# OATML-Markslab/ProteinGym

Hardware: AMD Instinct MI355X
Metric: mutants scored/sec (ESM-1v 650M masked-marginal) (higher is better)
Workload: dtype f16x3 (fp32 operands split into 2 fp16 planes, 3 fp16 MFMAs per product, fp32 accumulate)

## Files before the change

proteingym_amd/csrc/gemm16x_kernel.h:

```cpp
#pragma once
#include <type_traits>

#include "common.h"

namespace pgmi {

typedef _Float16 h8 __attribute__((ext_vector_type(8)));
typedef _Float16 h4 __attribute__((ext_vector_type(4)));
typedef __bf16 b8 __attribute__((ext_vector_type(8)));
typedef unsigned int u32x4 __attribute__((ext_vector_type(4)));
typedef unsigned int u32x2 __attribute__((ext_vector_type(2)));

__device__ __forceinline__ f32x4 gelu_erf16(f32x4 x) {
    auto all = [](float v) { return f32x4{v, v, v, v}; };
    const f32x4 b = __builtin_elementwise_max(-__builtin_elementwise_abs(x), all(-6.0f));
    f32x4 q = __builtin_elementwise_fma(x, all(0.0f), all(3.309269596e-05f));
    q = __builtin_elementwise_fma(q, b, all(7.692188374e-04f));
    q = __builtin_elementwise_fma(q, b, all(8.080714382e-03f));
    q = __builtin_elementwise_fma(q, b, all(5.341210216e-02f));
    q = __builtin_elementwise_fma(q, b, all(-4.587709904e-01f));
    q = __builtin_elementwise_fma(q, b, all(1.151201725e+00f));
    q = __builtin_elementwise_fma(q, b, all(-9.999930859e-01f));
    const f32x4 e = {__builtin_amdgcn_exp2f(q[0]), __builtin_amdgcn_exp2f(q[1]), __builtin_amdgcn_exp2f(q[2]), __builtin_amdgcn_exp2f(q[3])};
    return __builtin_elementwise_fma(b, e, __builtin_elementwise_max(x, all(0.0f)));
}

__device__ __forceinline__ f32x4 gelu_tanh16(f32x4 x) {
    constexpr float c = -2.0f * 0.7978845608028654f * 1.4426950408889634f;
    f32x4 r;
#pragma unroll
    for (int e = 0; e < 4; ++e) {
        const float u = fmaf(0.044715f * x[e], x[e] * x[e], x[e]);
        r[e] = x[e] / (1.0f + __builtin_amdgcn_exp2f(c * u));
    }
    return r;
}

struct QkvOut {
    unsigned short* vt16;
    size_t vt_plane;
    const float* cos_t;
    const float* sin_t;
    int T, H, Tp, rotary;
    int rot_halves;
};

template <bool BF>
__device__ __forceinline__ f32x16 mfma16(u32x4 a, u32x4 b, f32x16 c) {
    if constexpr (BF) {
        return __builtin_amdgcn_mfma_f32_32x32x16_bf16(__builtin_bit_cast(b8, a), __builtin_bit_cast(b8, b), c, 0, 0, 0);
    } else {
        return __builtin_amdgcn_mfma_f32_32x32x16_f16(__builtin_bit_cast(h8, a), __builtin_bit_cast(h8, b), c, 0, 0, 0);
    }
}

__device__ __forceinline__ unsigned short f32_to_bf16_rne(float f) {
    unsigned int u = __builtin_bit_cast(unsigned int, f);
    u += 0x7fffu + ((u >> 16) & 1u);
    return (unsigned short)(u >> 16);
}

struct TilePlan {
    int tiles_m, tiles_n;
    int n_main;
    int n_tail;
    int half;
    int group_m;
};

struct XMap {
    unsigned int a_row_bytes, w_row_bytes;
    unsigned int a_bytes, w_bytes;
    int k_run_log2;
    unsigned int a_run_bytes, w_run_bytes;
    int tiles_per_batch, batch_inner;
    unsigned int a_b0, a_b1, w_b0, w_b1;
    long long c_b0, c_b1;
    int ldc;
    int o_ld;
    int o_rows_per_n64;
    int o_col_per_batch;
};

constexpr int XBM = 256, XBN = 256, XNT = 512, XCPR = 8;
constexpr int X_OP_CH = XBM * XCPR;
constexpr int X_STAGE = 2 * X_OP_CH;
constexpr int X_PATCH_BYTES = 72 * 1024;
constexpr size_t X_LDS_BYTES = (size_t)(X_STAGE * 16 + X_PATCH_BYTES);

__device__ __forceinline__ void x_tile_coords(int wgid, int tiles_m, int tiles_n, int& tm, int& tn, int GROUP_M) {
    const int width = GROUP_M * tiles_n;
    const int group = wgid / width, first_m = group * GROUP_M;
    const int gsz = min(tiles_m - first_m, GROUP_M);
    tm = first_m + (wgid % width) % gsz;
    tn = (wgid % width) / gsz;
}

template <int EPI, int OUT, bool XM = false, bool BF = false>
__global__ __launch_bounds__(XNT, 2) void gemm16x_kernel(
    const unsigned short* __restrict__ A, const unsigned short* __restrict__ W, const float* __restrict__ bias,
    const float* residual, float* Cf, unsigned short* Ch, size_t c_plane, int M, int N, int K, float out_scale,
    TilePlan tp, QkvOut qo, XMap xm_arg) {
    static_assert(!(XM && BF), "the batched / strided form is f16x3 only");
    constexpr unsigned int EB = BF ? 2u : 4u;
    const XMap xm = XM ? xm_arg : XMap{};
    constexpr int WN = 4, TMX = 4, TN = 2, LD = 4;
    extern __shared__ __attribute__((aligned(16))) u32x4 lds[];
    const int tid = threadIdx.x, lane = tid & 63;
    const int wave = __builtin_amdgcn_readfirstlane(tid >> 6);
    const int wm = wave / WN, wn = wave % WN;
    const int r = lane & 31, kh = lane >> 5;
    const bool late = wave >= 4;
    unsigned char* const patches = reinterpret_cast<unsigned char*>(lds + X_STAGE);

    const int row_lo = tid >> 3, c8 = tid & 7, sw8 = (row_lo >> 1) & 7;
    const int csrc = c8 ^ sw8;
    const unsigned int a_row_bytes = xm.a_row_bytes ? xm.a_row_bytes : (unsigned int)K * EB;
    const unsigned int w_row_bytes = xm.w_row_bytes ? xm.w_row_bytes : (unsigned int)K * EB;
    const __amdgpu_buffer_rsrc_t rsA = __builtin_amdgcn_make_buffer_rsrc(const_cast<unsigned short*>(A), 0, (int)(xm.a_bytes ? xm.a_bytes : (unsigned int)M * (unsigned int)K * EB), 0x00020000);
    const __amdgpu_buffer_rsrc_t rsW = __builtin_amdgcn_make_buffer_rsrc(const_cast<unsigned short*>(W), 0, (int)(xm.w_bytes ? xm.w_bytes : (unsigned int)N * (unsigned int)K * EB), 0x00020000);
    unsigned int a_off[LD], w_off[LD];
    int m0 = 0, n0 = 0, a_ld = LD, batch = 0;
    unsigned int a_base = 0, w_base = 0;
    bool half_item = false;
    const int nk = BF ? K / 64 : K / 32;
    const int n_items = tp.n_main + tp.n_tail;
    auto decode = [&](int item) {
        const bool all_half = tp.half == 2;
        int wgid;
        if (item < tp.n_main || all_half) {
            const int nwg = all_half ? n_items : tp.n_main, xcd = item & 7, q = nwg >> 3, r8 = nwg & 7;
            wgid = (xcd < r8 ? xcd * (q + 1) : r8 * (q + 1) + (xcd - r8) * q) + (item >> 3);
        } else {
            wgid = tp.n_main + ((item - tp.n_main) >> 1);
        }
        batch = 0;
        if (xm.tiles_per_batch) {
            batch = wgid / xm.tiles_per_batch;
            wgid -= batch * xm.tiles_per_batch;
            const int bi = batch % xm.batch_inner, bo = batch / xm.batch_inner;
            a_base = __builtin_amdgcn_readfirstlane((unsigned int)bi * xm.a_b0 + (unsigned int)bo * xm.a_b1);
            w_base = __builtin_amdgcn_readfirstlane((unsigned int)bi * xm.w_b0 + (unsigned int)bo * xm.w_b1);
            batch = __builtin_amdgcn_readfirstlane(batch);
        }
        int tm, tn;
        x_tile_coords(wgid, tp.tiles_m, tp.tiles_n, tm, tn, tp.group_m);
        half_item = all_half || (tp.half && item >= tp.n_main);
        a_ld = half_item ? LD / 2 : LD;
        m0 = __builtin_amdgcn_readfirstlane(all_half ? tm * (XBM / 2) : tm * XBM + (half_item ? ((item - tp.n_main) & 1) * (XBM / 2) : 0));
        n0 = __builtin_amdgcn_readfirstlane(tn * XBN);
#pragma unroll
        for (int i = 0; i < LD; ++i) {
            a_off[i] = (unsigned int)min(m0 + row_lo + 64 * i, M - 1) * a_row_bytes + (unsigned int)csrc * 16u;
            w_off[i] = (unsigned int)min(n0 + row_lo + 64 * i, N - 1) * w_row_bytes + (unsigned int)csrc * 16u;
        }
    };
    auto issue_tile = [&](int kt, int buf) {
        u32x4* base = lds + buf * X_STAGE + wave * 64;
        const int run = kt >> xm.k_run_log2, in_run = kt - (run << xm.k_run_log2);
        const int ka = (int)(a_base + (xm.a_run_bytes ? (unsigned int)run * xm.a_run_bytes + (unsigned int)in_run * 128u : (unsigned int)kt * 128u));
        const int kw = (int)(w_base + (xm.w_run_bytes ? (unsigned int)run * xm.w_run_bytes + (unsigned int)in_run * 128u : (unsigned int)kt * 128u));
#pragma unroll
        for (int i = 0; i < LD; ++i)
            if (i < a_ld)
                __builtin_amdgcn_raw_ptr_buffer_load_lds(rsA, (__attribute__((address_space(3))) void*)(base + XNT * i), 16, (int)a_off[i], ka, 0, 0);
#pragma unroll
        for (int i = 0; i < LD; ++i)
            __builtin_amdgcn_raw_ptr_buffer_load_lds(rsW, (__attribute__((address_space(3))) void*)(base + X_OP_CH + XNT * i), 16, (int)w_off[i], kw, 0, 0);
    };
    auto phase = [&]() {
        __builtin_amdgcn_sched_barrier(0);
        __builtin_amdgcn_s_waitcnt(0xC07F);
        __builtin_amdgcn_s_barrier();
        __builtin_amdgcn_sched_barrier(0);
    };
    auto phase_vm = [&]() {
        __builtin_amdgcn_sched_barrier(0);
        __builtin_amdgcn_s_waitcnt(0x0070);
        __builtin_amdgcn_s_barrier();
        __builtin_amdgcn_sched_barrier(0);
    };

    f32x16 acc[TN][TMX];
    u32x4 af[2][TMX], wf[2][TN], whs[TN];
    const int fsw = (r >> 1) & 7;
    auto read_frags = [&](auto tmc, const u32x4* Ab, const u32x4* Wb, int ks) {
        constexpr int TM = decltype(tmc)::value;
#pragma unroll
        for (int p = 0; p < 2; ++p) {
            const int c = (p * 4 + ks * 2 + kh) ^ fsw;
#pragma unroll
            for (int i = 0; i < TM; ++i) af[p][i] = Ab[((wm * TM + i) * 32 + r) * XCPR + c];
#pragma unroll
            for (int j = 0; j < TN; ++j) wf[p][j] = Wb[((wn * TN + j) * 32 + r) * XCPR + c];
        }
    };
    auto scale_whi = [&]() {
        typedef _Float16 h2 __attribute__((ext_vector_type(2)));
        const h2 sc = {(_Float16)(1.0f / kLoScale), (_Float16)(1.0f / kLoScale)};
#pragma unroll
        for (int j = 0; j < TN; ++j)
#pragma unroll
            for (int e = 0; e < 4; ++e) {
                const unsigned int u = wf[0][j][e];
                const h2 t = __builtin_bit_cast(h2, u) * sc;
                whs[j][e] = __builtin_bit_cast(unsigned int, t);
            }
    };
    auto mfmas = [&](auto tmc) {
        constexpr int TM = decltype(tmc)::value;
        if constexpr (BF) {
#pragma unroll
            for (int p = 0; p < 2; ++p)
#pragma unroll
                for (int j = 0; j < TN; ++j)
#pragma unroll
                    for (int i = 0; i < TM; ++i) acc[j][i] = mfma16<true>(wf[p][j], af[p][i], acc[j][i]);
            return;
        }
        scale_whi();
#pragma unroll
        for (int j = 0; j < TN; ++j)
#pragma unroll
            for (int i = 0; i < TM; ++i) acc[j][i] = mfma16<false>(wf[1][j], af[0][i], acc[j][i]);
#pragma unroll
        for (int j = 0; j < TN; ++j)
#pragma unroll
            for (int i = 0; i < TM; ++i) acc[j][i] = mfma16<false>(whs[j], af[1][i], acc[j][i]);
#pragma unroll
        for (int j = 0; j < TN; ++j)
#pragma unroll
            for (int i = 0; i < TM; ++i) acc[j][i] = mfma16<false>(wf[0][j], af[0][i], acc[j][i]);
#pragma unroll
        for (int k = 0; k < 8; ++k) {
            __builtin_amdgcn_sched_group_barrier(0x008, 1, 0);
            __builtin_amdgcn_sched_group_barrier(0x002, 1, 0);
        }
        __builtin_amdgcn_sched_group_barrier(0x008, 3 * TN * TM - 8, 0);
    };

    int item = blockIdx.x;
    if (item >= n_items) return;
    decode(item);
    issue_tile(0, 0);
    auto run_item = [&](auto tmc) -> bool {
        constexpr int TM = decltype(tmc)::value;
        phase_vm();
#pragma unroll
        for (int j = 0; j < TN; ++j)
#pragma unroll
            for (int i = 0; i < TM; ++i)
#pragma unroll
                for (int v = 0; v < 16; ++v) acc[j][i][v] = 0.0f;
        int cur = 0;
        if (late) phase();
        for (int kt = 0; kt < nk; ++kt) {
            const u32x4* Ab = lds + cur * X_STAGE;
            const u32x4* Wb = Ab + X_OP_CH;
            __builtin_amdgcn_s_setprio(0);
            if (kt + 1 < nk) issue_tile(kt + 1, cur ^ 1);
            read_frags(tmc, Ab, Wb, 0);
            phase();
            __builtin_amdgcn_s_setprio(1);
            mfmas(tmc);
            phase();
            __builtin_amdgcn_s_setprio(0);
            read_frags(tmc, Ab, Wb, 1);
            if (late) phase_vm(); else phase();
            __builtin_amdgcn_s_setprio(1);
            mfmas(tmc);
            if (!late) phase_vm(); else phase();
            cur ^= 1;
        }
        __builtin_amdgcn_s_setprio(0);
        if (!late) phase();

        const int em0 = m0, en0 = n0, eb = batch;
        item += gridDim.x;
        const bool more = item < n_items;
        if (more) {
            decode(item);
            issue_tile(0, 0);
        }

        if constexpr (OUT == 2) {
            const int Dm = N / 3;
            const int nb = en0 + wn * 64;
            if (nb < N) {
            const int which = nb / Dm, hcol = nb - which * Dm, hh = hcol >> 6;
            constexpr int SPQ = 144;
            unsigned char* patch_q = patches + wave * (2 * 32 * SPQ);
            const bool staged_q = which < 2;
            f32x4 bq0[4], bq1[4];
#pragma unroll
            for (int g = 0; g < 4; ++g) {
                bq0[g] = *reinterpret_cast<const f32x4*>(bias + nb + 8 * g + 4 * kh);
                bq1[g] = *reinterpret_cast<const f32x4*>(bias + nb + 32 + 8 * g + 4 * kh);
            }
#pragma unroll
            for (int g = 0; g < 4; ++g) asm volatile("" :: "v"(bq0[g]), "v"(bq1[g]));
#pragma unroll
            for (int i = 0; i < TM; ++i) {
                const int m = em0 + (wm * TM + i) * 32 + r;
                const bool row_ok = m < M;
                if (!staged_q && !row_ok) continue;
                const int bb = m / qo.T, t = m - bb * qo.T;
                f32x4 rc[4], rs[4];
                if (which < 2 && qo.rotary) {
                    const int tr = (min(t, qo.T - 1) * qo.rot_halves + (hh % qo.rot_halves)) * 64;
#pragma unroll
                    for (int g = 0; g < 4; ++g) {
                        rc[g] = *reinterpret_cast<const f32x4*>(qo.cos_t + tr + 8 * g + 4 * kh);
                        rs[g] = *reinterpret_cast<const f32x4*>(qo.sin_t + tr + 8 * g + 4 * kh);
                    }
                }
                if (row_ok)
#pragma unroll
                for (int g = 0; g < 4; ++g) {
                    const int d0 = 8 * g + 4 * kh;
                    const f32x4 b0 = bq0[g], b1 = bq1[g];
                    float x0[4], x1[4];
#pragma unroll
                    for (int e = 0; e < 4; ++e) {
                        x0[e] = fmaf(acc[0][i][4 * g + e], out_scale, b0[e]);
                        x1[e] = fmaf(acc[1][i][4 * g + e], out_scale, b1[e]);
                    }
                    if (which == 0) {
#pragma unroll
                        for (int e = 0; e < 4; ++e) { x0[e] *= kQLog2e; x1[e] *= kQLog2e; }
                    }
                    if (which < 2) {
                        if (qo.rotary) {
                            const f32x4 c1 = rc[g], s1 = rs[g], c2 = rc[g], s2 = rs[g];
#pragma unroll
                            for (int e = 0; e < 4; ++e) {
                                const float y0 = fmaf(x0[e], c1[e], (-x1[e]) * s1[e]);
                                const float y1 = fmaf(x1[e], c2[e], x0[e] * s2[e]);
                                x0[e] = y0;
                                x1[e] = y1;
                            }
                        }
                        h4 hi0, lo0, hi1, lo1;
#pragma unroll
                        for (int e = 0; e < 4; ++e) {
                            _Float16 a, b2;
                            split_act(x0[e], a, b2); hi0[e] = a; lo0[e] = b2;
                            split_act(x1[e], a, b2); hi1[e] = a; lo1[e] = b2;
                        }
                        unsigned char* cell = patch_q + r * SPQ + d0 * 2;
                        *reinterpret_cast<h4*>(cell) = hi0;
                        *reinterpret_cast<h4*>(cell + 32 * SPQ) = lo0;
                        *reinterpret_cast<h4*>(cell + 64) = hi1;
                        *reinterpret_cast<h4*>(cell + 32 * SPQ + 64) = lo1;
                    } else {
                        const int tk = t & 31;
                        const int pos = (t & ~31) + ((tk & 0x13) | ((tk & 4) << 1) | ((tk & 8) >> 1));
                        unsigned short* col = qo.vt16 + (((size_t)bb * qo.H + hh) * kHeadDim + d0) * qo.Tp + pos;
#pragma unroll
                        for (int e = 0; e < 4; ++e) {
                            _Float16 a0, l0, a1, l1;
                            split_act(x0[e], a0, l0);
                            split_act(x1[e], a1, l1);
                            unsigned short* c0 = col + (size_t)e * qo.Tp;
                            unsigned short* c1p = c0 + (size_t)32 * qo.Tp;
                            c0[0] = __builtin_bit_cast(unsigned short, a0);
                            c0[qo.vt_plane] = __builtin_bit_cast(unsigned short, l0);
                            c1p[0] = __builtin_bit_cast(unsigned short, a1);
                            c1p[qo.vt_plane] = __builtin_bit_cast(unsigned short, l1);
                        }
                    }
                }
                if (staged_q) {
                    __builtin_amdgcn_wave_barrier();
                    const int m_base = em0 + (wm * TM + i) * 32;
#pragma unroll
                    for (int k = 0; k < 4; ++k) {
                        const int q = lane + 64 * k, row = q >> 3, cc = q & 7;
                        const u32x4 vh = *reinterpret_cast<const u32x4*>(patch_q + row * SPQ + cc * 16);
                        const u32x4 vl = *reinterpret_cast<const u32x4*>(patch_q + (32 + row) * SPQ + cc * 16);
                        if (m_base + row < M) {
                            unsigned short* dst = Ch + (size_t)(m_base + row) * (2 * Dm) + (size_t)which * Dm + hcol + cc * 8;
                            *reinterpret_cast<u32x4*>(dst) = vh;
                            *reinterpret_cast<u32x4*>(dst + c_plane) = vl;
                        }
                    }
                    __builtin_amdgcn_wave_barrier();
                }
            }
            }
        } else if constexpr (OUT == 0) {
            unsigned char* patch = patches + wave * (32 * 128);
            const int cc = lane & 7, rq = lane >> 3;
            const unsigned int kOob = 0x80000000u;
            const unsigned int ldc = xm.ldc ? (unsigned int)xm.ldc : (unsigned int)N;
            const long long cb = xm.tiles_per_batch ? (long long)(eb % xm.batch_inner) * xm.c_b0 + (long long)(eb / xm.batch_inner) * xm.c_b1 : 0;
            const __amdgpu_buffer_rsrc_t rsC = __builtin_amdgcn_make_buffer_rsrc(Cf + cb, 0, (int)((unsigned int)M * ldc * 4u), 0x00020000);
            const __amdgpu_buffer_rsrc_t rsR = __builtin_amdgcn_make_buffer_rsrc(const_cast<float*>(residual ? residual : Cf) + cb, 0, (int)((unsigned int)M * ldc * 4u), 0x00020000);
            unsigned int coff[TN];
            f32x4 bv[TN];
#pragma unroll
            for (int j = 0; j < TN; ++j) {
                const int n = en0 + (wn * TN + j) * 32 + cc * 4;
                coff[j] = n < N ? (unsigned int)n * 4u : kOob;
                bv[j] = (bias && n < N) ? *reinterpret_cast<const f32x4*>(bias + n) : f32x4{0.f, 0.f, 0.f, 0.f};
            }
#pragma unroll
            for (int j = 0; j < TN; ++j) asm volatile("" :: "v"(bv[j]));
            auto c_off = [&](int m, int j) -> int {
                return (int)((m < M && coff[j] != kOob) ? (unsigned int)m * ldc * 4u + coff[j] : kOob);
            };
            u32x4 rv[2][TN][4];
            auto load_residual = [&](int i, u32x4 (&dst)[TN][4]) {
                const int m_base = em0 + (wm * TM + i) * 32;
#pragma unroll
                for (int j = 0; j < TN; ++j)
#pragma unroll
                    for (int k = 0; k < 4; ++k)
                        dst[j][k] = __builtin_bit_cast(u32x4, __builtin_amdgcn_raw_buffer_load_b128(rsR, c_off(m_base + rq + 8 * k, j), 0, 0));
            };
            if (residual) load_residual(0, rv[0]);
#pragma unroll
            for (int i = 0; i < TM; ++i) {
                const int m_base = em0 + (wm * TM + i) * 32;
                if (residual && i + 1 < TM) load_residual(i + 1, rv[(i + 1) & 1]);
#pragma unroll
                for (int j = 0; j < TN; ++j) {
#pragma unroll
                    for (int g = 0; g < 4; ++g)
                        *reinterpret_cast<f32x4*>(patch + r * 128 + (((2 * g + kh) ^ (r & 7)) << 4)) =
                            f32x4{acc[j][i][4 * g], acc[j][i][4 * g + 1], acc[j][i][4 * g + 2], acc[j][i][4 * g + 3]};
                    __builtin_amdgcn_wave_barrier();
#pragma unroll
                    for (int k = 0; k < 4; ++k) {
                        const int row = rq + 8 * k;
                        const f32x4 a = *reinterpret_cast<const f32x4*>(patch + row * 128 + ((cc ^ (row & 7)) << 4));
                        f32x4 val;
#pragma unroll
                        for (int e = 0; e < 4; ++e) val[e] = fmaf(a[e], out_scale, bv[j][e]);
                        if (EPI == EPI_GELU) val = gelu_erf16(val);
                        if (EPI == EPI_GELU_TANH) val = gelu_tanh16(val);
                        if (EPI == EPI_SQRELU)
#pragma unroll
                        for (int e = 0; e < 4; ++e) { const float t = fmaxf(val[e], 0.0f); val[e] = t * t; }
                        if (residual) {
                            const f32x4 rr = __builtin_bit_cast(f32x4, rv[i & 1][j][k]);
#pragma unroll
                            for (int e = 0; e < 4; ++e) val[e] = rr[e] + val[e];
                        }
                        __builtin_amdgcn_raw_buffer_store_b128(__builtin_bit_cast(u32x4, val), rsC, c_off(m_base + row, j), 0, 0);
                    }
                    __builtin_amdgcn_wave_barrier();
                }
            }
        } else {
            if constexpr (BF) {
                constexpr int SPB = 144;
                const bool staged = (N % 8 == 0) && (en0 + (wn * TN + TN) * 32 <= N);
                unsigned char* patch = patches + wave * (32 * SPB);
                f32x4 bvs[TN][4];
#pragma unroll
                for (int j = 0; j < TN; ++j)
#pragma unroll
                    for (int g = 0; g < 4; ++g) {
                        const int n = en0 + (wn * TN + j) * 32 + 8 * g + 4 * kh;
                        bvs[j][g] = (bias && n < N) ? *reinterpret_cast<const f32x4*>(bias + n) : f32x4{0.f, 0.f, 0.f, 0.f};
                    }
#pragma unroll
                for (int j = 0; j < TN; ++j)
#pragma unroll
                    for (int g = 0; g < 4; ++g) asm volatile("" :: "v"(bvs[j][g]));
#pragma unroll
                for (int i = 0; i < TM; ++i) {
                    const int m = em0 + (wm * TM + i) * 32 + r;
                    const bool row_ok = m < M;
                    if (!staged && !row_ok) continue;
                    if (row_ok)
#pragma unroll
                    for (int j = 0; j < TN; ++j)
#pragma unroll
                        for (int g = 0; g < 4; ++g) {
                            const int n = en0 + (wn * TN + j) * 32 + 8 * g + 4 * kh;
                            if (n >= N) continue;
                            const f32x4 bv = bvs[j][g];
                            f32x4 val;
#pragma unroll
                            for (int e = 0; e < 4; ++e) val[e] = fmaf(acc[j][i][4 * g + e], out_scale, bv[e]);
                            if (EPI == EPI_GELU) val = gelu_erf16(val);
                            if (EPI == EPI_GELU_TANH) val = gelu_tanh16(val);
                            if (EPI == EPI_SQRELU)
#pragma unroll
                            for (int e = 0; e < 4; ++e) { const float t = fmaxf(val[e], 0.0f); val[e] = t * t; }
                            u32x2 pk;
                            pk[0] = (unsigned int)f32_to_bf16_rne(val[0]) | ((unsigned int)f32_to_bf16_rne(val[1]) << 16);
                            pk[1] = (unsigned int)f32_to_bf16_rne(val[2]) | ((unsigned int)f32_to_bf16_rne(val[3]) << 16);
                            if (staged) *reinterpret_cast<u32x2*>(patch + r * SPB + j * 64 + (8 * g + 4 * kh) * 2) = pk;
                            else *reinterpret_cast<u32x2*>(Ch + (size_t)m * (size_t)N + n) = pk;
                        }
                    if (staged) {
                        __builtin_amdgcn_wave_barrier();
                        const int m_base = em0 + (wm * TM + i) * 32;
                        const size_t ncol0 = (size_t)en0 + (size_t)wn * TN * 32;
#pragma unroll
                        for (int k = 0; k < 4; ++k) {
                            const int q = lane + 64 * k, row = q >> 3, cc = q & 7;
                            const u32x4 v = *reinterpret_cast<const u32x4*>(patch + row * SPB + cc * 16);
                            if (m_base + row < M) *reinterpret_cast<u32x4*>(Ch + (size_t)(m_base + row) * (size_t)N + ncol0 + cc * 8) = v;
                        }
                        __builtin_amdgcn_wave_barrier();
                    }
                }
            } else {
            constexpr int SP = 272;
            const bool staged = (N % 8 == 0) && (en0 + (wn * TN + TN) * 32 <= N);
            unsigned char* patch = patches + wave * (32 * SP);
            f32x4 bvs[TN][4];
#pragma unroll
            for (int j = 0; j < TN; ++j)
#pragma unroll
                for (int g = 0; g < 4; ++g) {
                    const int n = en0 + (wn * TN + j) * 32 + 8 * g + 4 * kh;
                    bvs[j][g] = (bias && n < N) ? *reinterpret_cast<const f32x4*>(bias + n) : f32x4{0.f, 0.f, 0.f, 0.f};
                }
#pragma unroll
            for (int j = 0; j < TN; ++j)
#pragma unroll
                for (int g = 0; g < 4; ++g) asm volatile("" :: "v"(bvs[j][g]));
#pragma unroll
            for (int i = 0; i < TM; ++i) {
                const int m = em0 + (wm * TM + i) * 32 + r;
                const bool row_ok = m < M;
                if (!staged && !row_ok) continue;
                if (row_ok)
#pragma unroll
                for (int j = 0; j < TN; ++j) {
#pragma unroll
                    for (int g = 0; g < 4; ++g) {
                        const int n = en0 + (wn * TN + j) * 32 + 8 * g + 4 * kh;
                        if (n >= N) continue;
                        const f32x4 bv = bvs[j][g];
                        f32x4 val;
#pragma unroll
                        for (int e = 0; e < 4; ++e) val[e] = fmaf(acc[j][i][4 * g + e], out_scale, bv[e]);
                        if (EPI == EPI_GELU) val = gelu_erf16(val);
                        if (EPI == EPI_GELU_TANH) val = gelu_tanh16(val);
                        if (EPI == EPI_SQRELU)
#pragma unroll
                        for (int e = 0; e < 4; ++e) { const float t = fmaxf(val[e], 0.0f); val[e] = t * t; }
                        {
                            h4 hi, lo;
#pragma unroll
                            for (int e = 0; e < 4; ++e) {
                                _Float16 a, b;
                                split_act(val[e], a, b);
                                hi[e] = a;
                                lo[e] = b;
                            }
                            if (staged) {
                                unsigned char* cell = patch + r * SP + j * 128 + (8 * g + 4 * kh) * 2;
                                *reinterpret_cast<h4*>(cell) = hi;
                                *reinterpret_cast<h4*>(cell + 64) = lo;
                            } else {
                                unsigned short* dst = Ch + ki_off((size_t)m, n, N);
                                *reinterpret_cast<h4*>(dst) = hi;
                                *reinterpret_cast<h4*>(dst + 32) = lo;
                            }
                        }
                    }
                }
                if (staged) {
                    __builtin_amdgcn_wave_barrier();
                    const int m_base = em0 + (wm * TM + i) * 32;
                    const size_t ncol0 = (size_t)en0 + (size_t)wn * TN * 32;
#pragma unroll
                    for (int k = 0; k < 8; ++k) {
                        const int q = lane + 64 * k;
                        const int row = q >> 4, cc = q & 15;
                        const u32x4 v = *reinterpret_cast<const u32x4*>(patch + row * SP + cc * 16);
                        if (m_base + row < M) {
                            if (xm.o_ld)
                                *reinterpret_cast<u32x4*>(Ch + ((size_t)(m_base + row) + (ncol0 >> 6) * (size_t)xm.o_rows_per_n64) * (2 * (size_t)xm.o_ld) +
                                                          (size_t)eb * (size_t)xm.o_col_per_batch * 2 + cc * 8) = v;
                            else
                                *reinterpret_cast<u32x4*>(Ch + (size_t)(m_base + row) * (2 * (size_t)N) + ncol0 * 2 + cc * 8) = v;
                        }
                    }
                    __builtin_amdgcn_wave_barrier();
                }
            }
            }
        }
        return more;
    };
    using Full = std::integral_constant<int, TMX>;
    using Half = std::integral_constant<int, TMX / 2>;
    while (true) {
        bool more;
        if constexpr (OUT != 2) more = half_item ? run_item(Half{}) : run_item(Full{});
        else more = run_item(Full{});
        if (!more) break;
    }
}

}
```

Baseline: 17660.

## Switch GEMM inner product from 32x32x16 to 16x16x32 MFMA tiles

Replaces the 32x32x16 f16/bf16 MFMA with the 16x16x32 variant, doubling the per-wave tile counts (TM 4→8, TN 2→4) so each wave covers the same output footprint, and splits each K-step into two halves over M sub-tiles instead of two K sub-steps. Fragment reads, scheduling group barriers and all epilogues (QKV rotary, residual, GELU, bf16 staging) are remapped to the 16-lane row/quad layout. Goal is better MFMA throughput or latency hiding with smaller instructions. The cost is more instructions and more fragment registers, plus an epilogue rework that could change staging correctness or bank conflicts.

Result: faster. 18360, median of 6 (+3.9%).

```diff
diff --git a/proteingym_amd/csrc/gemm16x_kernel.h b/proteingym_amd/csrc/gemm16x_kernel.h
--- a/proteingym_amd/csrc/gemm16x_kernel.h
+++ b/proteingym_amd/csrc/gemm16x_kernel.h
@@ -52,6 +52,20 @@
     } else {
         return __builtin_amdgcn_mfma_f32_32x32x16_f16(__builtin_bit_cast(h8, a), __builtin_bit_cast(h8, b), c, 0, 0, 0);
     }
+}
+
+template <bool BF>
+__device__ __forceinline__ f32x4 mfma16x16(u32x4 a, u32x4 b, f32x4 c) {
+    if constexpr (BF) {
+        return __builtin_amdgcn_mfma_f32_16x16x32_bf16(__builtin_bit_cast(b8, a), __builtin_bit_cast(b8, b), c, 0, 0, 0);
+    } else {
+        return __builtin_amdgcn_mfma_f32_16x16x32_f16(__builtin_bit_cast(h8, a), __builtin_bit_cast(h8, b), c, 0, 0, 0);
+    }
+}
+
+template <typename T>
+__device__ __forceinline__ void lds_put(unsigned char* p, T v) {
+    *(__attribute__((address_space(3))) T*)(p) = v;
 }
 
 __device__ __forceinline__ unsigned short f32_to_bf16_rne(float f) {
@@ -104,12 +118,12 @@
     static_assert(!(XM && BF), "the batched / strided form is f16x3 only");
     constexpr unsigned int EB = BF ? 2u : 4u;
     const XMap xm = XM ? xm_arg : XMap{};
-    constexpr int WN = 4, TMX = 4, TN = 2, LD = 4;
+    constexpr int WN = 4, TMX = 8, TN = 4, LD = 4;
     extern __shared__ __attribute__((aligned(16))) u32x4 lds[];
     const int tid = threadIdx.x, lane = tid & 63;
     const int wave = __builtin_amdgcn_readfirstlane(tid >> 6);
     const int wm = wave / WN, wn = wave % WN;
-    const int r = lane & 31, kh = lane >> 5;
+    const int r = lane & 15, kq = lane >> 4;
     const bool late = wave >= 4;
     unsigned char* const patches = reinterpret_cast<unsigned char*>(lds + X_STAGE);
 
@@ -181,18 +195,19 @@
         __builtin_amdgcn_sched_barrier(0);
     };
 
-    f32x16 acc[TN][TMX];
-    u32x4 af[2][TMX], wf[2][TN], whs[TN];
+    f32x4 acc[TN][TMX];
+    u32x4 af[2][TMX / 2], wf[2][TN], whs[TN];
     const int fsw = (r >> 1) & 7;
-    auto read_frags = [&](auto tmc, const u32x4* Ab, const u32x4* Wb, int ks) {
-        constexpr int TM = decltype(tmc)::value;
+    auto read_frags = [&](auto tmc, auto hc, const u32x4* Ab, const u32x4* Wb) {
+        constexpr int TM = decltype(tmc)::value, TH = TM / 2, H = decltype(hc)::value;
 #pragma unroll
         for (int p = 0; p < 2; ++p) {
-            const int c = (p * 4 + ks * 2 + kh) ^ fsw;
-#pragma unroll
-            for (int i = 0; i < TM; ++i) af[p][i] = Ab[((wm * TM + i) * 32 + r) * XCPR + c];
-#pragma unroll
-            for (int j = 0; j < TN; ++j) wf[p][j] = Wb[((wn * TN + j) * 32 + r) * XCPR + c];
+            const int c = (p * 4 + kq) ^ fsw;
+#pragma unroll
+            for (int i = 0; i < TH; ++i) af[p][i] = Ab[((wm * TM + H * TH + i) * 16 + r) * XCPR + c];
+            if constexpr (H == 0)
+#pragma unroll
+                for (int j = 0; j < TN; ++j) wf[p][j] = Wb[((wn * TN + j) * 16 + r) * XCPR + c];
         }
     };
     auto scale_whi = [&]() {
@@ -207,37 +222,41 @@
                 whs[j][e] = __builtin_bit_cast(unsigned int, t);
             }
     };
-    auto mfmas = [&](auto tmc) {
-        constexpr int TM = decltype(tmc)::value;
+    auto mfmas = [&](auto tmc, auto hc) {
+        constexpr int TM = decltype(tmc)::value, TH = TM / 2, H = decltype(hc)::value;
         if constexpr (BF) {
 #pragma unroll
             for (int p = 0; p < 2; ++p)
 #pragma unroll
                 for (int j = 0; j < TN; ++j)
 #pragma unroll
-                    for (int i = 0; i < TM; ++i) acc[j][i] = mfma16<true>(wf[p][j], af[p][i], acc[j][i]);
+                    for (int i = 0; i < TH; ++i) acc[j][H * TH + i] = mfma16x16<true>(wf[p][j], af[p][i], acc[j][H * TH + i]);
             return;
         }
-        scale_whi();
+        if constexpr (H == 0) scale_whi();
 #pragma unroll
         for (int j = 0; j < TN; ++j)
 #pragma unroll
-            for (int i = 0; i < TM; ++i) acc[j][i] = mfma16<false>(wf[1][j], af[0][i], acc[j][i]);
+            for (int i = 0; i < TH; ++i) acc[j][H * TH + i] = mfma16x16<false>(wf[1][j], af[0][i], acc[j][H * TH + i]);
 #pragma unroll
         for (int j = 0; j < TN; ++j)
 #pragma unroll
-            for (int i = 0; i < TM; ++i) acc[j][i] = mfma16<false>(whs[j], af[1][i], acc[j][i]);
+            for (int i = 0; i < TH; ++i) acc[j][H * TH + i] = mfma16x16<false>(whs[j], af[1][i], acc[j][H * TH + i]);
 #pragma unroll
         for (int j = 0; j < TN; ++j)
 #pragma unroll
-            for (int i = 0; i < TM; ++i) acc[j][i] = mfma16<false>(wf[0][j], af[0][i], acc[j][i]);
-#pragma unroll
-        for (int k = 0; k < 8; ++k) {
-            __builtin_amdgcn_sched_group_barrier(0x008, 1, 0);
-            __builtin_amdgcn_sched_group_barrier(0x002, 1, 0);
-        }
-        __builtin_amdgcn_sched_group_barrier(0x008, 3 * TN * TM - 8, 0);
-    };
+            for (int i = 0; i < TH; ++i) acc[j][H * TH + i] = mfma16x16<false>(wf[0][j], af[0][i], acc[j][H * TH + i]);
+        if constexpr (H == 0) {
+#pragma unroll
+            for (int k = 0; k < 4 * TN; ++k) {
+                __builtin_amdgcn_sched_group_barrier(0x008, 1, 0);
+                __builtin_amdgcn_sched_group_barrier(0x002, 1, 0);
+            }
+            __builtin_amdgcn_sched_group_barrier(0x008, 3 * TN * TH - 4 * TN, 0);
+        }
+    };
+    using H0 = std::integral_constant<int, 0>;
+    using H1 = std::integral_constant<int, 1>;
 
     int item = blockIdx.x;
     if (item >= n_items) return;
@@ -251,7 +270,7 @@
 #pragma unroll
             for (int i = 0; i < TM; ++i)
 #pragma unroll
-                for (int v = 0; v < 16; ++v) acc[j][i][v] = 0.0f;
+                for (int v = 0; v < 4; ++v) acc[j][i][v] = 0.0f;
         int cur = 0;
         if (late) phase();
         for (int kt = 0; kt < nk; ++kt) {
@@ -259,16 +278,16 @@
             const u32x4* Wb = Ab + X_OP_CH;
             __builtin_amdgcn_s_setprio(0);
             if (kt + 1 < nk) issue_tile(kt + 1, cur ^ 1);
-            read_frags(tmc, Ab, Wb, 0);
+            read_frags(tmc, H0{}, Ab, Wb);
             phase();
             __builtin_amdgcn_s_setprio(1);
-            mfmas(tmc);
+            mfmas(tmc, H0{});
             phase();
             __builtin_amdgcn_s_setprio(0);
-            read_frags(tmc, Ab, Wb, 1);
+            read_frags(tmc, H1{}, Ab, Wb);
             if (late) phase_vm(); else phase();
             __builtin_amdgcn_s_setprio(1);
-            mfmas(tmc);
+            mfmas(tmc, H1{});
             if (!late) phase_vm(); else phase();
             cur ^= 1;
         }
@@ -291,39 +310,41 @@
             constexpr int SPQ = 144;
             unsigned char* patch_q = patches + wave * (2 * 32 * SPQ);
             const bool staged_q = which < 2;
-            f32x4 bq0[4], bq1[4];
-#pragma unroll
-            for (int g = 0; g < 4; ++g) {
-                bq0[g] = *reinterpret_cast<const f32x4*>(bias + nb + 8 * g + 4 * kh);
-                bq1[g] = *reinterpret_cast<const f32x4*>(bias + nb + 32 + 8 * g + 4 * kh);
-            }
-#pragma unroll
-            for (int g = 0; g < 4; ++g) asm volatile("" :: "v"(bq0[g]), "v"(bq1[g]));
-#pragma unroll
-            for (int i = 0; i < TM; ++i) {
-                const int m = em0 + (wm * TM + i) * 32 + r;
+            f32x4 bq0[2], bq1[2];
+#pragma unroll
+            for (int g = 0; g < 2; ++g) {
+                bq0[g] = *reinterpret_cast<const f32x4*>(bias + nb + 16 * g + 4 * kq);
+                bq1[g] = *reinterpret_cast<const f32x4*>(bias + nb + 32 + 16 * g + 4 * kq);
+            }
+#pragma unroll
+            for (int g = 0; g < 2; ++g) asm volatile("" :: "v"(bq0[g]), "v"(bq1[g]));
+#pragma unroll
+            for (int ib = 0; ib < TM / 2; ++ib) {
+#pragma unroll
+            for (int s = 0; s < 2; ++s) {
+                const int i = 2 * ib + s, prow = 16 * s + r;
+                const int m = em0 + (wm * TM + i) * 16 + r;
                 const bool row_ok = m < M;
-                if (!staged_q && !row_ok) continue;
+                if (!row_ok) continue;
                 const int bb = m / qo.T, t = m - bb * qo.T;
-                f32x4 rc[4], rs[4];
+                f32x4 rc[2], rs[2];
                 if (which < 2 && qo.rotary) {
                     const int tr = (min(t, qo.T - 1) * qo.rot_halves + (hh % qo.rot_halves)) * 64;
 #pragma unroll
-                    for (int g = 0; g < 4; ++g) {
-                        rc[g] = *reinterpret_cast<const f32x4*>(qo.cos_t + tr + 8 * g + 4 * kh);
-                        rs[g] = *reinterpret_cast<const f32x4*>(qo.sin_t + tr + 8 * g + 4 * kh);
-                    }
-                }
-                if (row_ok)
-#pragma unroll
-                for (int g = 0; g < 4; ++g) {
-                    const int d0 = 8 * g + 4 * kh;
+                    for (int g = 0; g < 2; ++g) {
+                        rc[g] = *reinterpret_cast<const f32x4*>(qo.cos_t + tr + 16 * g + 4 * kq);
+                        rs[g] = *reinterpret_cast<const f32x4*>(qo.sin_t + tr + 16 * g + 4 * kq);
+                    }
+                }
+#pragma unroll
+                for (int g = 0; g < 2; ++g) {
+                    const int d0 = 16 * g + 4 * kq;
                     const f32x4 b0 = bq0[g], b1 = bq1[g];
                     float x0[4], x1[4];
 #pragma unroll
                     for (int e = 0; e < 4; ++e) {
-                        x0[e] = fmaf(acc[0][i][4 * g + e], out_scale, b0[e]);
-                        x1[e] = fmaf(acc[1][i][4 * g + e], out_scale, b1[e]);
+                        x0[e] = fmaf(acc[g][i][e], out_scale, b0[e]);
+                        x1[e] = fmaf(acc[g + 2][i][e], out_scale, b1[e]);
                     }
                     if (which == 0) {
 #pragma unroll
@@ -347,11 +368,11 @@
                             split_act(x0[e], a, b2); hi0[e] = a; lo0[e] = b2;
                             split_act(x1[e], a, b2); hi1[e] = a; lo1[e] = b2;
                         }
-                        unsigned char* cell = patch_q + r * SPQ + d0 * 2;
-                        *reinterpret_cast<h4*>(cell) = hi0;
-                        *reinterpret_cast<h4*>(cell + 32 * SPQ) = lo0;
-                        *reinterpret_cast<h4*>(cell + 64) = hi1;
-                        *reinterpret_cast<h4*>(cell + 32 * SPQ + 64) = lo1;
+                        unsigned char* cell = patch_q + prow * SPQ + d0 * 2;
+                        lds_put(cell, hi0);
+                        lds_put(cell + 32 * SPQ, lo0);
+                        lds_put(cell + 64, hi1);
+                        lds_put(cell + 32 * SPQ + 64, lo1);
                     } else {
                         const int tk = t & 31;
                         const int pos = (t & ~31) + ((tk & 0x13) | ((tk & 4) << 1) | ((tk & 8) >> 1));
@@ -370,9 +391,10 @@
                         }
                     }
                 }
+            }
                 if (staged_q) {
                     __builtin_amdgcn_wave_barrier();
-                    const int m_base = em0 + (wm * TM + i) * 32;
+                    const int m_base = em0 + (wm * TM + 2 * ib) * 16;
 #pragma unroll
                     for (int k = 0; k < 4; ++k) {
                         const int q = lane + 64 * k, row = q >> 3, cc = q & 7;
@@ -396,39 +418,43 @@
             const long long cb = xm.tiles_per_batch ? (long long)(eb % xm.batch_inner) * xm.c_b0 + (long long)(eb / xm.batch_inner) * xm.c_b1 : 0;
             const __amdgpu_buffer_rsrc_t rsC = __builtin_amdgcn_make_buffer_rsrc(Cf + cb, 0, (int)((unsigned int)M * ldc * 4u), 0x00020000);
             const __amdgpu_buffer_rsrc_t rsR = __builtin_amdgcn_make_buffer_rsrc(const_cast<float*>(residual ? residual : Cf) + cb, 0, (int)((unsigned int)M * ldc * 4u), 0x00020000);
-            unsigned int coff[TN];
-            f32x4 bv[TN];
-#pragma unroll
-            for (int j = 0; j < TN; ++j) {
-                const int n = en0 + (wn * TN + j) * 32 + cc * 4;
+            constexpr int NB = TN / 2;
+            unsigned int coff[NB];
+            f32x4 bv[NB];
+#pragma unroll
+            for (int j = 0; j < NB; ++j) {
+                const int n = en0 + wn * 64 + j * 32 + cc * 4;
                 coff[j] = n < N ? (unsigned int)n * 4u : kOob;
                 bv[j] = (bias && n < N) ? *reinterpret_cast<const f32x4*>(bias + n) : f32x4{0.f, 0.f, 0.f, 0.f};
             }
 #pragma unroll
-            for (int j = 0; j < TN; ++j) asm volatile("" :: "v"(bv[j]));
+            for (int j = 0; j < NB; ++j) asm volatile("" :: "v"(bv[j]));
             auto c_off = [&](int m, int j) -> int {
                 return (int)((m < M && coff[j] != kOob) ? (unsigned int)m * ldc * 4u + coff[j] : kOob);
             };
-            u32x4 rv[2][TN][4];
-            auto load_residual = [&](int i, u32x4 (&dst)[TN][4]) {
-                const int m_base = em0 + (wm * TM + i) * 32;
-#pragma unroll
-                for (int j = 0; j < TN; ++j)
+            u32x4 rv[2][NB][4];
+            auto load_residual = [&](int i, u32x4 (&dst)[NB][4]) {
+                const int m_base = em0 + (wm * TM + 2 * i) * 16;
+#pragma unroll
+                for (int j = 0; j < NB; ++j)
 #pragma unroll
                     for (int k = 0; k < 4; ++k)
                         dst[j][k] = __builtin_bit_cast(u32x4, __builtin_amdgcn_raw_buffer_load_b128(rsR, c_off(m_base + rq + 8 * k, j), 0, 0));
             };
             if (residual) load_residual(0, rv[0]);
 #pragma unroll
-            for (int i = 0; i < TM; ++i) {
-                const int m_base = em0 + (wm * TM + i) * 32;
-                if (residual && i + 1 < TM) load_residual(i + 1, rv[(i + 1) & 1]);
-#pragma unroll
-                for (int j = 0; j < TN; ++j) {
-#pragma unroll
-                    for (int g = 0; g < 4; ++g)
-                        *reinterpret_cast<f32x4*>(patch + r * 128 + (((2 * g + kh) ^ (r & 7)) << 4)) =
-                            f32x4{acc[j][i][4 * g], acc[j][i][4 * g + 1], acc[j][i][4 * g + 2], acc[j][i][4 * g + 3]};
+            for (int i = 0; i < TM / 2; ++i) {
+                const int m_base = em0 + (wm * TM + 2 * i) * 16;
+                if (residual && i + 1 < TM / 2) load_residual(i + 1, rv[(i + 1) & 1]);
+#pragma unroll
+                for (int j = 0; j < NB; ++j) {
+#pragma unroll
+                    for (int s = 0; s < 2; ++s)
+#pragma unroll
+                        for (int u = 0; u < 2; ++u) {
+                            const int prow = 16 * s + r;
+                            *reinterpret_cast<f32x4*>(patch + prow * 128 + (((4 * u + kq) ^ (prow & 7)) << 4)) = acc[2 * j + u][2 * i + s];
+                        }
                     __builtin_amdgcn_wave_barrier();
 #pragma unroll
                     for (int k = 0; k < 4; ++k) {
@@ -455,36 +481,31 @@
         } else {
             if constexpr (BF) {
                 constexpr int SPB = 144;
-                const bool staged = (N % 8 == 0) && (en0 + (wn * TN + TN) * 32 <= N);
+                const bool staged = (N % 8 == 0) && (en0 + (wn + 1) * 64 <= N);
                 unsigned char* patch = patches + wave * (32 * SPB);
-                f32x4 bvs[TN][4];
-#pragma unroll
-                for (int j = 0; j < TN; ++j)
-#pragma unroll
-                    for (int g = 0; g < 4; ++g) {
-                        const int n = en0 + (wn * TN + j) * 32 + 8 * g + 4 * kh;
-                        bvs[j][g] = (bias && n < N) ? *reinterpret_cast<const f32x4*>(bias + n) : f32x4{0.f, 0.f, 0.f, 0.f};
-                    }
-#pragma unroll
-                for (int j = 0; j < TN; ++j)
-#pragma unroll
-                    for (int g = 0; g < 4; ++g) asm volatile("" :: "v"(bvs[j][g]));
-#pragma unroll
-                for (int i = 0; i < TM; ++i) {
-                    const int m = em0 + (wm * TM + i) * 32 + r;
-                    const bool row_ok = m < M;
-                    if (!staged && !row_ok) continue;
-                    if (row_ok)
-#pragma unroll
-                    for (int j = 0; j < TN; ++j)
-#pragma unroll
-                        for (int g = 0; g < 4; ++g) {
-                            const int n = en0 + (wn * TN + j) * 32 + 8 * g + 4 * kh;
+                f32x4 bvs[TN];
+#pragma unroll
+                for (int j = 0; j < TN; ++j) {
+                    const int n = en0 + wn * 64 + 16 * j + 4 * kq;
+                    bvs[j] = (bias && n < N) ? *reinterpret_cast<const f32x4*>(bias + n) : f32x4{0.f, 0.f, 0.f, 0.f};
+                }
+#pragma unroll
+                for (int j = 0; j < TN; ++j) asm volatile("" :: "v"(bvs[j]));
+#pragma unroll
+                for (int ib = 0; ib < TM / 2; ++ib) {
+#pragma unroll
+                    for (int s = 0; s < 2; ++s) {
+                    const int i = 2 * ib + s, prow = 16 * s + r;
+                    const int m = em0 + (wm * TM + i) * 16 + r;
+                    if (m >= M) continue;
+#pragma unroll
+                    for (int j = 0; j < TN; ++j) {
+                            const int n = en0 + wn * 64 + 16 * j + 4 * kq;
                             if (n >= N) continue;
-                            const f32x4 bv = bvs[j][g];
+                            const f32x4 bv = bvs[j];
                             f32x4 val;
 #pragma unroll
-                            for (int e = 0; e < 4; ++e) val[e] = fmaf(acc[j][i][4 * g + e], out_scale, bv[e]);
+                            for (int e = 0; e < 4; ++e) val[e] = fmaf(acc[j][i][e], out_scale, bv[e]);
                             if (EPI == EPI_GELU) val = gelu_erf16(val);
                             if (EPI == EPI_GELU_TANH) val = gelu_tanh16(val);
                             if (EPI == EPI_SQRELU)
@@ -493,13 +514,14 @@
                             u32x2 pk;
                             pk[0] = (unsigned int)f32_to_bf16_rne(val[0]) | ((unsigned int)f32_to_bf16_rne(val[1]) << 16);
                             pk[1] = (unsigned int)f32_to_bf16_rne(val[2]) | ((unsigned int)f32_to_bf16_rne(val[3]) << 16);
-                            if (staged) *reinterpret_cast<u32x2*>(patch + r * SPB + j * 64 + (8 * g + 4 * kh) * 2) = pk;
+                            if (staged) lds_put(patch + prow * SPB + (16 * j + 4 * kq) * 2, pk);
                             else *reinterpret_cast<u32x2*>(Ch + (size_t)m * (size_t)N + n) = pk;
                         }
+                    }
                     if (staged) {
                         __builtin_amdgcn_wave_barrier();
-                        const int m_base = em0 + (wm * TM + i) * 32;
-                        const size_t ncol0 = (size_t)en0 + (size_t)wn * TN * 32;
+                        const int m_base = em0 + (wm * TM + 2 * ib) * 16;
+                        const size_t ncol0 = (size_t)en0 + (size_t)wn * 64;
 #pragma unroll
                         for (int k = 0; k < 4; ++k) {
                             const int q = lane + 64 * k, row = q >> 3, cc = q & 7;
@@ -511,36 +533,33 @@
                 }
             } else {
             constexpr int SP = 272;
-            const bool staged = (N % 8 == 0) && (en0 + (wn * TN + TN) * 32 <= N);
+            const bool staged = (N % 8 == 0) && (en0 + (wn + 1) * 64 <= N);
             unsigned char* patch = patches + wave * (32 * SP);
-            f32x4 bvs[TN][4];
-#pragma unroll
-            for (int j = 0; j < TN; ++j)
-#pragma unroll
-                for (int g = 0; g < 4; ++g) {
-                    const int n = en0 + (wn * TN + j) * 32 + 8 * g + 4 * kh;
-                    bvs[j][g] = (bias && n < N) ? *reinterpret_cast<const f32x4*>(bias + n) : f32x4{0.f, 0.f, 0.f, 0.f};
-                }
-#pragma unroll
-            for (int j = 0; j < TN; ++j)
-#pragma unroll
-                for (int g = 0; g < 4; ++g) asm volatile("" :: "v"(bvs[j][g]));
-#pragma unroll
-            for (int i = 0; i < TM; ++i) {
-                const int m = em0 + (wm * TM + i) * 32 + r;
-                const bool row_ok = m < M;
-                if (!staged && !row_ok) continue;
-                if (row_ok)
+            f32x4 bvs[TN];
+#pragma unroll
+            for (int j = 0; j < TN; ++j) {
+                const int n = en0 + wn * 64 + 16 * j + 4 * kq;
+                bvs[j] = (bias && n < N) ? *reinterpret_cast<const f32x4*>(bias + n) : f32x4{0.f, 0.f, 0.f, 0.f};
+            }
+#pragma unroll
+            for (int j = 0; j < TN; ++j) asm volatile("" :: "v"(bvs[j]));
+#pragma unroll
+            for (int ib = 0; ib < TM / 2; ++ib) {
+#pragma unroll
+                for (int s = 0; s < 2; ++s) {
+                const int i = 2 * ib + s, prow = 16 * s + r;
+                const int m = em0 + (wm * TM + i) * 16 + r;
+                if (m >= M) continue;
 #pragma unroll
                 for (int j = 0; j < TN; ++j) {
-#pragma unroll
-                    for (int g = 0; g < 4; ++g) {
-                        const int n = en0 + (wn * TN + j) * 32 + 8 * g + 4 * kh;
+                    {
+                        const int c = 16 * j + 4 * kq;
+                        const int n = en0 + wn * 64 + c;
                         if (n >= N) continue;
-                        const f32x4 bv = bvs[j][g];
+                        const f32x4 bv = bvs[j];
                         f32x4 val;
 #pragma unroll
-                        for (int e = 0; e < 4; ++e) val[e] = fmaf(acc[j][i][4 * g + e], out_scale, bv[e]);
+                        for (int e = 0; e < 4; ++e) val[e] = fmaf(acc[j][i][e], out_scale, bv[e]);
                         if (EPI == EPI_GELU) val = gelu_erf16(val);
                         if (EPI == EPI_GELU_TANH) val = gelu_tanh16(val);
                         if (EPI == EPI_SQRELU)
@@ -556,9 +575,9 @@
                                 lo[e] = b;
                             }
                             if (staged) {
-                                unsigned char* cell = patch + r * SP + j * 128 + (8 * g + 4 * kh) * 2;
-                                *reinterpret_cast<h4*>(cell) = hi;
-                                *reinterpret_cast<h4*>(cell + 64) = lo;
+                                unsigned char* cell = patch + prow * SP + (c >> 5) * 128 + (c & 31) * 2;
+                                lds_put(cell, hi);
+                                lds_put(cell + 64, lo);
                             } else {
                                 unsigned short* dst = Ch + ki_off((size_t)m, n, N);
                                 *reinterpret_cast<h4*>(dst) = hi;
@@ -567,10 +586,11 @@
                         }
                     }
                 }
+                }
                 if (staged) {
                     __builtin_amdgcn_wave_barrier();
-                    const int m_base = em0 + (wm * TM + i) * 32;
-                    const size_t ncol0 = (size_t)en0 + (size_t)wn * TN * 32;
+                    const int m_base = em0 + (wm * TM + 2 * ib) * 16;
+                    const size_t ncol0 = (size_t)en0 + (size_t)wn * 64;
 #pragma unroll
                     for (int k = 0; k < 8; ++k) {
                         const int q = lane + 64 * k;
```
